# microsoft/Spartan

Measured on AMD Instinct MI355X. Metric: R1CS constraints/sec in SNARK::prove (synthetic 2^20); bit-exact proof, higher is better.
Workload: dtype u64x4 (F_q Montgomery / F_p 2^255-19 limbs)

## Files before the change

### profiles/fq_bandwidth.py

```python
#!/usr/bin/env python3
import csv, sqlite3, sys, collections, re
db = sqlite3.connect(sys.argv[1])
cols = [r[1] for r in db.execute("PRAGMA table_info(kernels)")]
low = {c.lower(): c for c in cols}
def pick(*names):
    for n in names:
        if n in low: return low[n]
    return None
gx, gy, gz = pick("grid_size_x", "grid_x"), pick("grid_size_y", "grid_y"), pick("grid_size_z", "grid_z")
gtot = pick("grid_size")
dcol = low.get("duration") or "(end - start)"
gexpr = gtot if gtot and not gx else "*".join(c for c in (gx, gy, gz) if c)
dur = collections.defaultdict(list)
for name, g, d in db.execute("select name, %s, %s from kernels" % (gexpr, dcol)):
    k = name.split("(")[0].replace("void ", "")
    dur[(k, int(g))].append(d / 1e3)
def load(path, counter):
    tot = collections.defaultdict(float); n = collections.Counter()
    rd = csv.DictReader(open(path))
    gcols = [c for c in rd.fieldnames if c.lower().startswith("grid_size")]
    for row in rd:
        if row["Counter_Name"] != counter: continue
        k = row["Kernel_Name"].split("(")[0].replace("void ", "")
        g = 1
        for c in gcols:
            try: g *= max(1, int(float(row[c])))
            except ValueError: pass
        tot[(k, g)] += float(row["Counter_Value"]); n[(k, g)] += 1
    return tot, n
f, nf = load(sys.argv[2], "FETCH_SIZE"); w, nw = load(sys.argv[3], "WRITE_SIZE")
res = {}
if len(sys.argv) > 4:
    for line in open(sys.argv[4]):
        m = re.match(r"(\S+)\s+vgprs\s+(\d+)\s+waves_per_simd\s+(\d+)", line)
        if m: res[m.group(1)] = (int(m.group(2)), int(m.group(3)))
sq = {}
if len(sys.argv) > 5:
    for c in ("SQ_ACTIVE_INST_VALU", "SQ_WAIT_INST_ANY", "SQ_WAVE_CYCLES"):
        try: sq[c] = load(sys.argv[5], c)
        except OSError: sq = {}; break
def sq_share(k, g, c):
    if not sq: return None
    num, nn = sq[c]; den, nd = sq["SQ_WAVE_CYCLES"]
    if not nn.get((k, g)) or not den.get((k, g)): return None
    return (num[(k, g)] / nn[(k, g)]) / (den[(k, g)] / nd[(k, g)])
FQ = ("k_sc_", "k_cubic_", "k_vecmat", "k_dot", "k_hash_layer", "k_eval_table", "k_sparse_eval", "k_eq_outer", "k_prod_layer", "k_gather", "k_evaluate", "k_spmv", "k_colsum", "k_bind_top", "k_from_index", "k_scale_prefix")
rows = []
for (k, g), ds in dur.items():
    if not k.startswith(FQ): continue
    fb = 2.0 * f.get((k, g), 0.0) * 1024 / max(nf.get((k, g), 1), 1)
    wb = w.get((k, g), 0.0) * 1024 / max(nw.get((k, g), 1), 1)
    avg = sorted(ds)[len(ds) // 2]
    rows.append((k, g, len(ds), avg, fb + wb))
print("# F_q kernels by launch size: HBM bytes per launch (PMC: 2 x FETCH_SIZE + WRITE_SIZE, KiB counters) / median duration (kernel trace)")
print("# throughput-sized = a launch that moves >= 64 MB; the rest is launch-sized (latency-bound by construction: its TB/s says nothing)")
hdr = "%-44s %10s %6s %10s %10s %8s  %-20s %s" % ("kernel", "grid", "calls", "median_us", "MB/launch", "TB/s", "vgprs/waves_per_simd", "valu  wait" if sq else "")
for title, sel in (("throughput-sized launches (>= 64 MB)", lambda r: r[4] >= 64e6), ("launch-sized (< 64 MB), the ten with the most total time", lambda r: r[4] < 64e6)):
    print("\n## " + title); print(hdr)
    part = [r for r in rows if sel(r)]
    part.sort(key=lambda r: -r[2] * r[3])
    if "launch-sized" in title: part = part[:10]
    for k, g, n, avg, b in part:
        base = k.split("<")[0]
        rv = res.get(k) or res.get(base)
        va, wa = sq_share(k, g, "SQ_ACTIVE_INST_VALU"), sq_share(k, g, "SQ_WAIT_INST_ANY")
        tail = ("%.2f  %.2f" % (va, wa)) if (va is not None and wa is not None) else ""
        print("%-44s %10d %6d %10.1f %10.1f %8.2f  %-20s %s" % (k[:44], g, n, avg, b / 1e6, b / avg / 1e6 if avg else 0.0, ("%d / %d" % rv) if rv else "-", tail))
tot_t = sum(r[2] * r[3] for r in rows if r[4] >= 64e6); tot_b = sum(r[2] * r[4] for r in rows if r[4] >= 64e6)
if tot_t: print("\n# all throughput-sized F_q launches together: %.1f ms, %.1f GB -> %.2f TB/s" % (tot_t / 1e3, tot_b / 1e9, tot_b / tot_t / 1e6))
```

### spartan_amd/csrc/field.hpp

```cpp
#pragma once
#include <cstdint>
#include <cstring>

#if defined(__HIPCC__)
#include <hip/hip_runtime.h>
#define SP_HD __host__ __device__ __forceinline__
#define SP_HD_NOINLINE __host__ __device__ __noinline__
#else
#define SP_HD inline
#define SP_HD_NOINLINE
#endif

namespace sp {

typedef unsigned __int128 u128;

struct Fq {
  uint64_t l[4];
};

#define SP_Q0 0x5812631a5cf5d3edULL
#define SP_Q1 0x14def9dea2f79cd6ULL
#define SP_Q2 0x0000000000000000ULL
#define SP_Q3 0x1000000000000000ULL
// ... 262 lines not shown
  }
  constexpr int nprod = i1 - i0 + 1;
  constexpr int nred = (has7 ? 1 : 0) + (K < 8 ? (K < 3 ? K : 3) : (K <= 10 ? 11 - K : 0));
  fq_terms<nprod + nred>(lo, hi, x, y);
  if (K < 8) {
    uint64_t t;
    asm("v_mad_u64_u32 %0, vcc, %1, %2, 0" : "=v"(t) : "v"((uint32_t)lo), "v"((uint32_t)SP_QINV) : "vcc");
    m[K] = (uint32_t)t;
    fq_term1(lo, hi, m[K], q[0]);
  } else {
    r[K - 8] = (uint32_t)lo;
  }
  lo = (lo >> 32) | ((uint64_t)hi << 32);
  hi = 0;
}
__device__ __forceinline__ Fq fq_mul(const Fq& A, const Fq& B) {
  uint32_t a[8], b[8], m[8], r[8];
#pragma unroll
  for (int i = 0; i < 4; i++) {
    a[2 * i] = (uint32_t)A.l[i]; a[2 * i + 1] = (uint32_t)(A.l[i] >> 32);
    b[2 * i] = (uint32_t)B.l[i]; b[2 * i + 1] = (uint32_t)(B.l[i] >> 32);
  }
  const uint32_t q[8] = {(uint32_t)SP_Q0, (uint32_t)(SP_Q0 >> 32), (uint32_t)SP_Q1, (uint32_t)(SP_Q1 >> 32), 0, 0, 0, (uint32_t)(SP_Q3 >> 32)};
  uint64_t lo = 0;
  uint32_t hi = 0;
  fq_column<0>(lo, hi, a, b, m, q, r); fq_column<1>(lo, hi, a, b, m, q, r); fq_column<2>(lo, hi, a, b, m, q, r); fq_column<3>(lo, hi, a, b, m, q, r);
  fq_column<4>(lo, hi, a, b, m, q, r); fq_column<5>(lo, hi, a, b, m, q, r); fq_column<6>(lo, hi, a, b, m, q, r); fq_column<7>(lo, hi, a, b, m, q, r);
  fq_column<8>(lo, hi, a, b, m, q, r); fq_column<9>(lo, hi, a, b, m, q, r); fq_column<10>(lo, hi, a, b, m, q, r); fq_column<11>(lo, hi, a, b, m, q, r);
  fq_column<12>(lo, hi, a, b, m, q, r); fq_column<13>(lo, hi, a, b, m, q, r); fq_column<14>(lo, hi, a, b, m, q, r);
  r[7] = (uint32_t)lo;
  Fq t = {{(uint64_t)r[0] | ((uint64_t)r[1] << 32), (uint64_t)r[2] | ((uint64_t)r[3] << 32), (uint64_t)r[4] | ((uint64_t)r[5] << 32),
           (uint64_t)r[6] | ((uint64_t)r[7] << 32)}};
  return fq_csub(t);
}
__host__ inline Fq fq_mul(const Fq& a, const Fq& b) {
#else
SP_HD Fq fq_mul(const Fq& a, const Fq& b) {
#endif
  uint64_t r[8] = {0, 0, 0, 0, 0, 0, 0, 0};
#pragma unroll
  for (int i = 0; i < 4; i++) {
    u128 c = 0;
#pragma unroll
    for (int j = 0; j < 4; j++) {
      c += (u128)a.l[i] * b.l[j] + r[i + j];
      r[i + j] = (uint64_t)c;
      c >>= 64;
    }
    r[i + 4] = (uint64_t)c;
  }
  return fq_mont_reduce(r);
}
SP_HD Fq fq_sqr(const Fq& a) { return fq_mul(a, a); }
SP_HD Fq fq_from_mont(const Fq& a) {
  uint64_t r[8] = {a.l[0], a.l[1], a.l[2], a.l[3], 0, 0, 0, 0};
  return fq_mont_reduce(r);
}
SP_HD Fq fq_to_mont(const Fq& canonical) { return fq_mul(canonical, fq_R2()); }
SP_HD Fq fq_from_u64(uint64_t v) { return fq_mul(Fq{{v, 0, 0, 0}}, fq_R2()); }
SP_HD Fq fq_from_u512(const uint64_t w[8]) {
  Fq d0 = {{w[0], w[1], w[2], w[3]}}, d1 = {{w[4], w[5], w[6], w[7]}};
  return fq_add(fq_mul(d0, fq_R2()), fq_mul(d1, fq_R3()));
}
SP_HD Fq fq_pow(const Fq& a, const uint64_t e[4]) {
  Fq res = fq_one();
  for (int w = 3; w >= 0; w--)
    for (int i = 63; i >= 0; i--) {
      res = fq_sqr(res);
      if ((e[w] >> i) & 1) res = fq_mul(res, a);
    }
  return res;
}
SP_HD Fq fq_invert(const Fq& a) {
  const uint64_t e[4] = {SP_Q0 - 2, SP_Q1, SP_Q2, SP_Q3};
  return fq_pow(a, e);
}

SP_HD Fq operator+(const Fq& a, const Fq& b) { return fq_add(a, b); }
SP_HD Fq operator-(const Fq& a, const Fq& b) { return fq_sub(a, b); }
SP_HD Fq operator*(const Fq& a, const Fq& b) { return fq_mul(a, b); }
SP_HD Fq operator-(const Fq& a) { return fq_neg(a); }
SP_HD bool operator==(const Fq& a, const Fq& b) { return fq_eq(a, b); }
SP_HD bool operator!=(const Fq& a, const Fq& b) { return !fq_eq(a, b); }
SP_HD Fq& operator+=(Fq& a, const Fq& b) { a = fq_add(a, b); return a; }
SP_HD Fq& operator-=(Fq& a, const Fq& b) { a = fq_sub(a, b); return a; }
SP_HD Fq& operator*=(Fq& a, const Fq& b) { a = fq_mul(a, b); return a; }

struct Fp {
  uint64_t v[4];
};

SP_HD Fp fp_zero() { return Fp{{0, 0, 0, 0}}; }
SP_HD Fp fp_one() { return Fp{{1, 0, 0, 0}}; }

SP_HD uint64_t fp_add_small(Fp& r, uint64_t x) {
  u128 c = (u128)r.v[0] + x;
  r.v[0] = (uint64_t)c;
  c >>= 64;
#pragma unroll
  for (int i = 1; i < 4; i++) {
    c += r.v[i];
    r.v[i] = (uint64_t)c;
    c >>= 64;
  }
  return (uint64_t)c;
}
// ... 270 lines not shown
```

### spartan_amd/csrc/fq_ops.hip

```cpp
#include "internal.hpp"

constexpr int EQ_TOPB = 4;
__device__ __forceinline__ Fq eq_suffix(const Fq* __restrict__ r, size_t ell, int topb, size_t lo) {
  Fq acc = fq_one();
  int nl = (int)ell - topb;
  for (int k = 0; k < nl; k++) {
    Fq rk = ld_fq(r + topb + k);
    bool bit = (lo >> (nl - 1 - k)) & 1;
    acc = fq_mul(acc, bit ? rk : fq_sub(fq_one(), rk));
  }
  return acc;
}
template <int TOPB>
__device__ __forceinline__ void eq_expand_top(Fq (&v)[1 << TOPB], const Fq* __restrict__ r, const Fq& suffix) {
  v[0] = suffix;
#pragma unroll
  for (int k = 0; k < TOPB; k++) {
    Fq rk = ld_fq(r + k);
#pragma unroll
    for (int i = (1 << k) - 1; i >= 0; i--) {
      Fq hi = fq_mul(v[i], rk);
      v[2 * i + 1] = hi;
      v[2 * i] = fq_sub(v[i], hi);
    }
// ... 167 lines not shown
  }
  __syncthreads();
  if (role < 3) {
    Fq e = fq_zero();
    if (live && (KIND == 2 || role < 2)) {
      Fq pt[4];
#pragma unroll
      for (int k = 0; k < NT; k++) {
        Fq x0 = bound[li][2 * k], x1 = bound[li][2 * k + 1];
        Fq x2 = fq_sub(fq_dbl(x1), x0), x3 = fq_sub(fq_add(x2, x1), x0);
#pragma unroll
        for (int w = 0; w < 4; w++) pt[k].l[w] = role == 0 ? x0.l[w] : (role == 1 ? x2.l[w] : x3.l[w]);
      }
      if (KIND == 0) e = fq_mul(pt[0], pt[1]);
      else e = fq_mul(pt[0], fq_sub(fq_mul(pt[1], pt[2]), pt[3]));
    }
    red[role][li] = e;
  }
  __syncthreads();
  for (int s = 16; s > 0; s >>= 1) {
    if (role < 3 && li < s) red[role][li] = fq_add(red[role][li], red[role][li + s]);
    __syncthreads();
  }
  if (threadIdx.x < 3) st_fq(partials + (size_t)blockIdx.x * 3 + threadIdx.x, red[threadIdx.x][0]);
  signal_done(sig);
}
__global__ void __launch_bounds__(256) k_bind_top(Tabs4 T, int ntabs, size_t half, Fq r) { SP_FG_PRIO();
  for (size_t i = (size_t)blockIdx.x * blockDim.x + threadIdx.x; i < half; i += (size_t)gridDim.x * blockDim.x) {
    for (int k = 0; k < ntabs; k++) {
      Fq x0 = ld_fq(T.p[k] + i), x1 = ld_fq(T.p[k] + half + i);
      st_fq(T.p[k] + i, fq_add(x0, fq_mul(r, fq_sub(x1, x0))));
    }
  }
}
__global__ void __launch_bounds__(256) k_reduce_partials(const Fq* __restrict__ partials, size_t nblk, int K, Fq* __restrict__ out, DoneSig sig) { SP_FG_PRIO();
  __shared__ Fq sm[256];
  for (int k = 0; k < K; k++) {
    Fq acc[1] = {fq_zero()};
    for (size_t b = threadIdx.x; b < nblk; b += 256) acc[0] = fq_add(acc[0], ld_fq(partials + b * K + k));
    block_sum_fq<1>(acc, sm);
    if (threadIdx.x == 0) st_fq(out + k, acc[0]);
  }
  signal_done(sig);
}
__global__ void __launch_bounds__(256) k_vecmat(const Fq* __restrict__ L, size_t Lsz, const Fq* __restrict__ Z, size_t R, size_t jchunk,
                                                Fq* __restrict__ partial) { SP_FG_PRIO();
  __shared__ Fq sm[4][64];
  const int cl = threadIdx.x & 63, g = threadIdx.x >> 6;
  size_t i = (size_t)blockIdx.x * 64 + cl;
  size_t j0 = (size_t)blockIdx.y * jchunk, j1 = j0 + jchunk;
  if (j1 > Lsz) j1 = Lsz;
  Fq acc = fq_zero();
  if (i < R)
    for (size_t j = j0 + g; j < j1; j += 4) acc = fq_add(acc, fq_mul(ld_fq(L + j), ld_fq(Z + j * R + i)));
  sm[g][cl] = acc;
  __syncthreads();
  if (g == 0 && i < R) st_fq(partial + (size_t)blockIdx.y * R + i, fq_add(fq_add(sm[0][cl], sm[1][cl]), fq_add(sm[2][cl], sm[3][cl])));
}
__global__ void __launch_bounds__(256) k_colsum(const Fq* __restrict__ partial, size_t nchunks, size_t R, Fq* __restrict__ out) { SP_FG_PRIO();
  __shared__ Fq sm[8][32];
  const int cl = threadIdx.x & 31, g = threadIdx.x >> 5;
  size_t i = (size_t)blockIdx.x * 32 + cl;
  Fq acc = fq_zero();
  if (i < R)
    for (size_t c = g; c < nchunks; c += 8) acc = fq_add(acc, ld_fq(partial + c * R + i));
  sm[g][cl] = acc;
  __syncthreads();
  for (int s = 4; s > 0; s >>= 1) {
    if (g < s) sm[g][cl] = fq_add(sm[g][cl], sm[g + s][cl]);
    __syncthreads();
  }
  if (g == 0 && i < R) st_fq(out + i, sm[0][cl]);
}
static size_t vecmat_jchunk(size_t Lsz, size_t R) { return Lsz * R <= ((size_t)1 << 22) ? 16 : 32; }
__global__ void __launch_bounds__(256) k_dot(const Fq* __restrict__ a, const Fq* __restrict__ b, size_t n, Fq* __restrict__ partials) { SP_FG_PRIO();
  __shared__ Fq sm[256];
  Fq acc[1] = {fq_zero()};
  for (size_t i = (size_t)blockIdx.x * blockDim.x + threadIdx.x; i < n; i += (size_t)gridDim.x * blockDim.x)
    acc[0] = fq_add(acc[0], fq_mul(ld_fq(a + i), ld_fq(b + i)));
  block_sum_fq<1>(acc, sm);
  if (threadIdx.x == 0) st_fq(partials + blockIdx.x, acc[0]);
}
__global__ void k_gather_elems(const Fq* const* __restrict__ ptrs, size_t n, size_t count, Fq* __restrict__ out) { SP_FG_PRIO();
  size_t t = (size_t)blockIdx.x * blockDim.x + threadIdx.x;
  if (t < n * count) st_fq(out + t, ld_fq(ptrs[t / count] + t % count));
}


static void host_sum(const Fq* p, size_t nblk, int K, uint64_t* out) {
  Fq* o = (Fq*)out;
  for (int k = 0; k < K; k++) {
    Fq acc = p[k];
    for (size_t b = 1; b < nblk; b++) acc = fq_add(acc, p[b * K + k]);
    o[k] = acc;
  }
}
int32_t reduce_and_fetch(sp_ctx* c, Fq* partials, size_t nblk, int K, uint64_t* out) {
  if (partials != (Fq*)hres(c)) {
    DoneSig sig = sig_make(c, 1);
    {
      ProfScope ps(c, PF_REDUCE, 32.0 * (double)(nblk * K));
      hipLaunchKernelGGL(k_reduce_partials, dim3(1), dim3(256), 0, c->stream, (const Fq*)partials, nblk, K, (Fq*)hres(c), sig);
    }
    SPCHK(sig_wait(c, sig));
    memcpy(out, hres(c), 32 * K);
    return hipGetLastError() == hipSuccess ? SP_OK : SP_EHIP;
  }
// ... 446 lines not shown
```

### spartan_amd/csrc/internal.hpp

```cpp
#pragma once
#include <hip/hip_runtime.h>

#include <cstdio>
#include <cstdlib>
#include <cstring>
#include <new>
#include <map>
#include <vector>

#include "../../include/spartan_hip.h"
#include "curve.hpp"
#include "field.hpp"
#include "msm.hpp"
#include "options.hpp"

using namespace sp;

enum ProfFamily {
  PF_GENS_TABLE = 0,
  PF_MSM_ROWS,
  PF_MSM_WINDOWS,
  PF_MSM_REDUCE_PASS,
  PF_MSM_REDUCE,
  PF_EQ_EXPAND,
// ... 234 lines not shown
int32_t reduce_and_fetch(sp_ctx* c, Fq* partials, size_t nblk, int K, uint64_t* out);
constexpr size_t SP_HOST_ENCODE_ROWS = 8;
extern "C" int32_t msm_launch(sp_ctx* c, const sp_gens* g, const Fq* dZ, size_t z_stride, size_t rows, size_t cols, size_t g_off,
                              const uint32_t* didx, const Fq* dblinds, size_t h_idx, uint8_t* out_host, size_t idx_row_stride = 0,
                              Pt* points_out = nullptr );

enum MsmRowsForm { MSM_ROWS_WINDOWS = 0, MSM_ROWS_STRIP, MSM_ROWS_FLAT };
size_t msm_flat_slots();
void msm_rows_enqueue(sp_ctx* c, hipStream_t st, const sp_gens* g, const Fq* dZ, size_t z_stride, size_t rows, size_t cols, size_t g_off,
                      const uint32_t* didx, const Fq* dblinds, size_t h_idx, Pt* partial, int form, size_t strip, size_t P);

size_t msm_lds_runs(const sp_gens* g, size_t rows, size_t cols, bool has_blinds, size_t wg_slots);
void msm_lds_enqueue(sp_ctx* c, hipStream_t st, const sp_gens* g, const Fq* dZ, size_t z_stride, size_t rows, size_t cols, size_t g_off,
                     const uint32_t* didx, const Fq* dblinds, size_t h_idx, Pt* partial, size_t nb, unsigned grid_limit);

struct MsmQRuns { unsigned nb, len, S; };
constexpr unsigned MSMQ_MAX_GROUPS = 1024, MSMQ_BLOCK_WORDS = 2 * MSMQ_MAX_GROUPS + 2 , MSMQ_BLOCKS = 256;
enum MsmQRole { MSMQ_ALONE = 0, MSMQ_CORESIDENT = 2 };
MsmQRuns msm_q_cut(const sp_ctx* c, const sp_gens* g, size_t rows, size_t cols, bool has_blinds, int role);
void msm_q_enqueue(sp_ctx* c, hipStream_t st, const sp_gens* g, const Fq* dZ, size_t z_stride, size_t rows, size_t cols, size_t g_off,
                   const uint32_t* didx, const Fq* dblinds, size_t h_idx, Pt* partial, const MsmQRuns& r, int role,
                   const unsigned** counts_out ,
                   const unsigned long long** issued_out );

static inline size_t grid_for(size_t work, size_t maxblocks = 2048) {
  size_t b = (work + 255) / 256;
  if (b < 1) b = 1;
  return b > maxblocks ? maxblocks : b;
}
static inline bool is_pow2(size_t x) { return x && !(x & (x - 1)); }
static inline size_t ilog2(size_t x) {
  size_t l = 0;
  while (((size_t)1 << l) < x) l++;
  return l;
}

#ifndef SP_FG_PRIO_OFF
#define SP_FG_PRIO() __builtin_amdgcn_s_setprio(3)
#else
#define SP_FG_PRIO() do { } while (0)
#endif

__device__ __forceinline__ Fq ld_fq(const Fq* p) {
  const ulonglong2* q = reinterpret_cast<const ulonglong2*>(p);
  ulonglong2 a = q[0], b = q[1];
  return Fq{{a.x, a.y, b.x, b.y}};
}
__device__ __forceinline__ void st_fq(Fq* p, const Fq& v) {
  ulonglong2* q = reinterpret_cast<ulonglong2*>(p);
  q[0] = make_ulonglong2(v.l[0], v.l[1]);
  q[1] = make_ulonglong2(v.l[2], v.l[3]);
}

template <int K>
__device__ __forceinline__ void block_sum_fq(Fq (&v)[K], Fq* smem ) {
  int t = threadIdx.x;
#pragma unroll
  for (int k = 0; k < K; k++) {
    __syncthreads();
    smem[t] = v[k];
    __syncthreads();
    for (int s = 128; s > 0; s >>= 1) {
      if (t < s) smem[t] = fq_add(smem[t], smem[t + s]);
      __syncthreads();
    }
    v[k] = smem[0];
  }
}


__global__ void k_reduce_partials(const Fq* __restrict__ partials, size_t nblk, int K, Fq* __restrict__ out);
```

### spartan_amd/csrc/spark.hip

```cpp
#include "internal.hpp"

__global__ void __launch_bounds__(256) k_from_index(const uint32_t* __restrict__ ix, size_t n, Fq* __restrict__ dst) { SP_FG_PRIO();
  for (size_t i = (size_t)blockIdx.x * blockDim.x + threadIdx.x; i < n; i += (size_t)gridDim.x * blockDim.x) st_fq(dst + i, fq_from_u64(ix[i]));
}
__global__ void __launch_bounds__(256) k_gather(const Fq* __restrict__ mem, const uint32_t* __restrict__ addr, size_t n, Fq* __restrict__ dst) { SP_FG_PRIO();
  for (size_t i = (size_t)blockIdx.x * blockDim.x + threadIdx.x; i < n; i += (size_t)gridDim.x * blockDim.x) st_fq(dst + i, ld_fq(mem + addr[i]));
}
__global__ void __launch_bounds__(256) k_hash_layer(const Fq* __restrict__ addr, const Fq* __restrict__ val, const Fq* __restrict__ ts, int ts_inc,
                                                    size_t n, Fq r_hash, Fq r_hash_sqr, Fq r_multiset, Fq* __restrict__ dst) { SP_FG_PRIO();
  for (size_t i = (size_t)blockIdx.x * blockDim.x + threadIdx.x; i < n; i += (size_t)gridDim.x * blockDim.x) {
    Fq a = addr ? ld_fq(addr + i) : fq_from_u64((uint64_t)i);
    Fq t = ts ? ld_fq(ts + i) : fq_zero();
    if (ts_inc) t = fq_add(t, fq_one());
    Fq h = fq_add(fq_add(fq_mul(t, r_hash_sqr), fq_mul(ld_fq(val + i), r_hash)), a);
    st_fq(dst + i, fq_sub(h, r_multiset));
  }
}
template <bool PAIR>
__global__ void __launch_bounds__(256) k_hash_layer_first(const Fq* __restrict__ addr, const Fq* __restrict__ val, const Fq* __restrict__ ts, int ts_inc,
                                                          size_t n, Fq r_hash, Fq r_hash_sqr, Fq r_multiset, Fq* __restrict__ dst_a, Fq* __restrict__ dst_b) { SP_FG_PRIO();
  const size_t half = n / 2;
  for (size_t i = (size_t)blockIdx.x * blockDim.x + threadIdx.x; i < half; i += (size_t)gridDim.x * blockDim.x) {
    Fq h[2];
#pragma unroll
    for (int k = 0; k < 2; k++) {
      const size_t j = i + (size_t)k * half;
      Fq a = addr ? ld_fq(addr + j) : fq_from_u64((uint64_t)j);
      Fq t = ts ? ld_fq(ts + j) : fq_zero();
      if (ts_inc) t = fq_add(t, fq_one());
      h[k] = fq_sub(fq_add(fq_add(fq_mul(t, r_hash_sqr), fq_mul(ld_fq(val + j), r_hash)), a), r_multiset);
      st_fq(dst_a + j, h[k]);
    }
    st_fq(dst_a + n + i, fq_mul(h[0], h[1]));
    if (PAIR) {
      Fq w0 = fq_add(h[0], r_hash_sqr), w1 = fq_add(h[1], r_hash_sqr);
      st_fq(dst_b + i, w0);
      st_fq(dst_b + half + i, w1);
      st_fq(dst_b + n + i, fq_mul(w0, w1));
    }
  }
}
__global__ void __launch_bounds__(256) k_prod_layer(const Fq* __restrict__ in, size_t half, Fq* __restrict__ out) { SP_FG_PRIO();
  for (size_t i = (size_t)blockIdx.x * blockDim.x + threadIdx.x; i < half; i += (size_t)gridDim.x * blockDim.x)
    st_fq(out + i, fq_mul(ld_fq(in + i), ld_fq(in + half + i)));
}

struct Stores16 {
  Fq* p[16];
};
__global__ void __launch_bounds__(256) k_prod_layer_many(Stores16 st, size_t off, size_t half, size_t noff) { SP_FG_PRIO();
  const Fq* in = st.p[blockIdx.y] + off;
  Fq* out = st.p[blockIdx.y] + noff;
  for (size_t i = (size_t)blockIdx.x * blockDim.x + threadIdx.x; i < half; i += (size_t)gridDim.x * blockDim.x)
    st_fq(out + i, fq_mul(ld_fq(in + i), ld_fq(in + half + i)));
}

__global__ void __launch_bounds__(256) k_prod_layer2_many(Stores16 st, size_t off, size_t len) { SP_FG_PRIO();
  const size_t q = len / 4, off1 = off + len, off2 = off1 + len / 2;
  Fq* base = st.p[blockIdx.y];
  for (size_t i = (size_t)blockIdx.x * blockDim.x + threadIdx.x; i < q; i += (size_t)gridDim.x * blockDim.x) {
    const Fq x0 = ld_fq(base + off + i), x1 = ld_fq(base + off + q + i), x2 = ld_fq(base + off + 2 * q + i), x3 = ld_fq(base + off + 3 * q + i);
    const Fq lo = fq_mul(x0, x2), hi = fq_mul(x1, x3);
    st_fq(base + off1 + i, lo);
    st_fq(base + off1 + q + i, hi);
    st_fq(base + off2 + i, fq_mul(lo, hi));
  }
}
__global__ void __launch_bounds__(256) k_prod_layer_tail(Stores16 st, size_t off, size_t len) { SP_FG_PRIO();
  __shared__ Fq cur[1024];
  Fq* base = st.p[blockIdx.x];
  size_t half = len / 2, noff = off + len;
  for (size_t i = threadIdx.x; i < half; i += 256) {
    Fq v = fq_mul(ld_fq(base + off + i), ld_fq(base + off + half + i));
    cur[i] = v;
    st_fq(base + noff + i, v);
  }
  __syncthreads();
  len = half;
  while (len > 2) {
    half = len / 2;
    noff += len;
    Fq v[2];
    int n = 0;
// ... 14 lines not shown
__device__ __forceinline__ void cubic_point(const Fq& a0, const Fq& a1, const Fq& b0, const Fq& b1, const Fq& c0, const Fq& c1, Fq (&e)[3]) {
  Fq da = fq_sub(a1, a0), db = fq_sub(b1, b0), dc = fq_sub(c1, c0);
  Fq a2 = fq_add(a1, da), b2 = fq_add(b1, db), c2 = fq_add(c1, dc);
  Fq a3 = fq_add(a2, da), b3 = fq_add(b2, db), c3 = fq_add(c2, dc);
  e[0] = fq_add(e[0], fq_mul(fq_mul(a0, b0), c0));
  e[1] = fq_add(e[1], fq_mul(fq_mul(a2, b2), c2));
  e[2] = fq_add(e[2], fq_mul(fq_mul(a3, b3), c3));
}
__global__ void __launch_bounds__(256) k_cubic_eval_batched(const Triple* __restrict__ T, TripleInline IN, size_t half, Fq* __restrict__ partials) { SP_FG_PRIO();
  __shared__ Fq sm[256];
  Triple t = T ? T[blockIdx.y] : IN.t[blockIdx.y];
  Fq e[3] = {fq_zero(), fq_zero(), fq_zero()};
  for (size_t i = (size_t)blockIdx.x * blockDim.x + threadIdx.x; i < half; i += (size_t)gridDim.x * blockDim.x)
    cubic_point(ld_fq(t.a + i), ld_fq(t.a + half + i), ld_fq(t.b + i), ld_fq(t.b + half + i), ld_fq(t.c + i), ld_fq(t.c + half + i), e);
  block_sum_fq<3>(e, sm);
  if (threadIdx.x == 0) {
    Fq* p = partials + ((size_t)blockIdx.y * gridDim.x + blockIdx.x) * 3;
    st_fq(p, e[0]); st_fq(p + 1, e[1]); st_fq(p + 2, e[2]);
  }
}
__global__ void __launch_bounds__(256) k_cubic_bind_eval_batched(const Triple* __restrict__ T, TripleInline IN, size_t quarter, Fq r, Fq* __restrict__ partials) { SP_FG_PRIO();
  __shared__ Fq sm[256];
  Triple t = T ? T[blockIdx.y] : IN.t[blockIdx.y];
  Fq e[3] = {fq_zero(), fq_zero(), fq_zero()};
  for (size_t i = (size_t)blockIdx.x * blockDim.x + threadIdx.x; i < quarter; i += (size_t)gridDim.x * blockDim.x) {
    Fq lo[3], hi[3];
    Fq* ptr[3] = {t.a, t.b, t.c};
#pragma unroll
    for (int k = 0; k < 3; k++) {
      Fq x0 = ld_fq(ptr[k] + i), x1 = ld_fq(ptr[k] + quarter + i), x2 = ld_fq(ptr[k] + 2 * quarter + i), x3 = ld_fq(ptr[k] + 3 * quarter + i);
      lo[k] = fq_add(x0, fq_mul(r, fq_sub(x2, x0)));
      hi[k] = fq_add(x1, fq_mul(r, fq_sub(x3, x1)));
      if (k < 2) {
        st_fq(ptr[k] + i, lo[k]);
        st_fq(ptr[k] + quarter + i, hi[k]);
      } else if (t.c_out) {
        st_fq(t.c_out + i, lo[k]);
        st_fq(t.c_out + quarter + i, hi[k]);
      }
    }
    cubic_point(lo[0], hi[0], lo[1], hi[1], lo[2], hi[2], e);
  }
  block_sum_fq<3>(e, sm);
  if (threadIdx.x == 0) {
    Fq* p = partials + ((size_t)blockIdx.y * gridDim.x + blockIdx.x) * 3;
    st_fq(p, e[0]); st_fq(p + 1, e[1]); st_fq(p + 2, e[2]);
  }
}
__device__ __forceinline__ void quad_point_eq(const Fq& a0, const Fq& a1, const Fq& b0, const Fq& b1, const Fq& c, Fq (&e)[4]) {
  Fq a2 = fq_add(a1, fq_sub(a1, a0)), b2 = fq_add(b1, fq_sub(b1, b0));
  e[0] = fq_add(e[0], fq_mul(fq_mul(a0, b0), c));
  e[1] = fq_add(e[1], fq_mul(fq_mul(a2, b2), c));
}
__device__ __forceinline__ void cubic_point4(const Fq& a0, const Fq& a1, const Fq& b0, const Fq& b1, const Fq& c0, const Fq& c1, Fq (&e)[4]) {
  Fq da = fq_sub(a1, a0), db = fq_sub(b1, b0), dc = fq_sub(c1, c0);
  Fq a2 = fq_add(a1, da), b2 = fq_add(b1, db), c2 = fq_add(c1, dc);
  Fq a3 = fq_add(a2, da), b3 = fq_add(b2, db), c3 = fq_add(c2, dc);
  e[0] = fq_add(e[0], fq_mul(fq_mul(a0, b0), c0));
  e[1] = fq_add(e[1], fq_mul(fq_mul(a1, b1), c1));
  e[2] = fq_add(e[2], fq_mul(fq_mul(a2, b2), c2));
  e[3] = fq_add(e[3], fq_mul(fq_mul(a3, b3), c3));
}
template <bool GEN>
__global__ void __launch_bounds__(256) k_cubic_eval_batched_eq(TripleInline IN, unsigned inst0, size_t half, Fq* __restrict__ partials) { SP_FG_PRIO();
  __shared__ Fq sm[256];
  const unsigned inst = inst0 + blockIdx.y;
  Triple t = IN.t[inst];
  Fq e[4] = {fq_zero(), fq_zero(), fq_zero(), fq_zero()};
  if (!GEN) {
    for (size_t i = (size_t)blockIdx.x * blockDim.x + threadIdx.x; i < half; i += (size_t)gridDim.x * blockDim.x)
      quad_point_eq(ld_fq(t.a + i), ld_fq(t.a + half + i), ld_fq(t.b + i), ld_fq(t.b + half + i), ld_fq(t.c + i), e);
  } else {
    for (size_t i = (size_t)blockIdx.x * blockDim.x + threadIdx.x; i < half; i += (size_t)gridDim.x * blockDim.x)
      cubic_point4(ld_fq(t.a + i), ld_fq(t.a + half + i), ld_fq(t.b + i), ld_fq(t.b + half + i), ld_fq(t.c + i), ld_fq(t.c + half + i), e);
  }
  if (GEN) block_sum_fq<4>(e, sm);
  else {
    Fq q[2] = {e[0], e[1]};
    block_sum_fq<2>(q, sm);
    e[0] = q[0]; e[1] = q[1];
  }
  if (threadIdx.x == 0) {
    Fq* p = partials + ((size_t)inst * gridDim.x + blockIdx.x) * 4;
    st_fq(p, e[0]); st_fq(p + 1, e[1]); st_fq(p + 2, e[2]); st_fq(p + 3, e[3]);
  }
}
template <bool GEN>
__global__ void __launch_bounds__(256) k_cubic_bind_eval_batched_eq(TripleInline IN, unsigned inst0, size_t quarter, Fq r, Fq* __restrict__ partials) { SP_FG_PRIO();
  __shared__ Fq sm[256];
  const unsigned inst = inst0 + blockIdx.y;
  Triple t = IN.t[inst];
  Fq e[4] = {fq_zero(), fq_zero(), fq_zero(), fq_zero()};
  for (size_t i = (size_t)blockIdx.x * blockDim.x + threadIdx.x; i < quarter; i += (size_t)gridDim.x * blockDim.x) {
    Fq lo[3], hi[3];
    Fq* ptr[3] = {t.a, t.b, t.c};
#pragma unroll
    for (int k = 0; k < 2; k++) {
      Fq x0 = ld_fq(ptr[k] + i), x1 = ld_fq(ptr[k] + quarter + i), x2 = ld_fq(ptr[k] + 2 * quarter + i), x3 = ld_fq(ptr[k] + 3 * quarter + i);
      lo[k] = fq_add(x0, fq_mul(r, fq_sub(x2, x0)));
      hi[k] = fq_add(x1, fq_mul(r, fq_sub(x3, x1)));
      st_fq(ptr[k] + i, lo[k]);
      st_fq(ptr[k] + quarter + i, hi[k]);
    }
    if (!GEN) {
      quad_point_eq(lo[0], hi[0], lo[1], hi[1], ld_fq(t.c + i), e);
    } else {
      Fq x0 = ld_fq(ptr[2] + i), x1 = ld_fq(ptr[2] + quarter + i), x2 = ld_fq(ptr[2] + 2 * quarter + i), x3 = ld_fq(ptr[2] + 3 * quarter + i);
      lo[2] = fq_add(x0, fq_mul(r, fq_sub(x2, x0)));
      hi[2] = fq_add(x1, fq_mul(r, fq_sub(x3, x1)));
      if (t.c_out) {
        st_fq(t.c_out + i, lo[2]);
        st_fq(t.c_out + quarter + i, hi[2]);
      }
      cubic_point4(lo[0], hi[0], lo[1], hi[1], lo[2], hi[2], e);
    }
  }
  if (GEN) block_sum_fq<4>(e, sm);
  else {
    Fq q[2] = {e[0], e[1]};
    block_sum_fq<2>(q, sm);
    e[0] = q[0]; e[1] = q[1];
  }
  if (threadIdx.x == 0) {
    Fq* p = partials + ((size_t)inst * gridDim.x + blockIdx.x) * 4;
// ... 150 lines not shown
    const int k = lane / 3, tt = lane % 3;
    const Fq P = lv[grp][k][2][tt], U = lv[grp][k][3][tt];
    lv[grp][k][4][tt] = fq_add(P, U);
    lv[grp][k][5][tt] = fq_sub(P, U);
  }
  __syncthreads();
  Fq e = fq_zero();
  if (live && lane < 18 && np >= 2) {
    const int tt = lane / 6, kind = lane % 6;
    if (kind == 0 || np == 4) {
      e = fq_mul(fq_mul(lv[grp][0][kind][tt], lv[grp][1][kind][tt]), lv[grp][2][kind][tt]);
      SP_KT(kt, 4);
      if (weights) e = fq_mul(e, wv);
    }
  }
  SP_KT(kt, 5);
  if (lane < 18) red[lane][grp] = e;
  __syncthreads();
  if (threadIdx.x < 18) {
    Fq acc = red[threadIdx.x][0];
#pragma unroll
    for (int k = 1; k < 8; k++) acc = fq_add(acc, red[threadIdx.x][k]);
    red[threadIdx.x][0] = acc;
  }
  __syncthreads();
  if (threadIdx.x < 18) {
    Fq* o = partials + ((size_t)blockIdx.y * gridDim.x + blockIdx.x) * 18;
    const int x = threadIdx.x;
    Fq v;
    if (x < 3) v = fq_add(red[6 * x][0], red[6 * x + 1][0]);
    else if (x < 15) v = red[6 * ((x - 3) / 4) + 2 + (x - 3) % 4][0];
    else v = (n2 == 1 && blockIdx.x == 0) ? bnd[0][(x - 15) * 4] : fq_zero();
    st_fq(o + x, v);
  }
  SP_KT(kt, 6);
  signal_done(sig);
  SP_KT(kt, 7);
}
__global__ void __launch_bounds__(256) k_reduce_partials_batched(const Fq* __restrict__ partials, size_t nblk, int K, Fq* __restrict__ out, DoneSig sig) { SP_FG_PRIO();
  __shared__ Fq sm[256];
  const Fq* p = partials + (size_t)blockIdx.x * nblk * K;
  for (int k = 0; k < K; k++) {
    Fq acc[1] = {fq_zero()};
    for (size_t b = threadIdx.x; b < nblk; b += 256) acc[0] = fq_add(acc[0], ld_fq(p + b * K + k));
    block_sum_fq<1>(acc, sm);
    if (threadIdx.x == 0) st_fq(out + (size_t)blockIdx.x * K + k, acc[0]);
  }
  signal_done(sig);
}
__global__ void __launch_bounds__(256) k_dot_many(const Fq* __restrict__ chi, Fq* const* __restrict__ tabs, size_t n, Fq* __restrict__ partials) { SP_FG_PRIO();
  __shared__ Fq sm[256];
  const Fq* t = tabs[blockIdx.y];
  Fq acc[1] = {fq_zero()};
  for (size_t i = (size_t)blockIdx.x * blockDim.x + threadIdx.x; i < n; i += (size_t)gridDim.x * blockDim.x)
    acc[0] = fq_add(acc[0], fq_mul(ld_fq(chi + i), ld_fq(t + i)));
  block_sum_fq<1>(acc, sm);
  if (threadIdx.x == 0) st_fq(partials + (size_t)blockIdx.y * gridDim.x + blockIdx.x, acc[0]);
}
__global__ void __launch_bounds__(256) k_dot3(const Fq* __restrict__ l, const Fq* __restrict__ r, const Fq* __restrict__ w, size_t n,
                                              Fq* __restrict__ partials) { SP_FG_PRIO();
  __shared__ Fq sm[256];
  Fq acc[1] = {fq_zero()};
  for (size_t i = (size_t)blockIdx.x * blockDim.x + threadIdx.x; i < n; i += (size_t)gridDim.x * blockDim.x)
    acc[0] = fq_add(acc[0], fq_mul(fq_mul(ld_fq(l + i), ld_fq(r + i)), ld_fq(w + i)));
  block_sum_fq<1>(acc, sm);
  if (threadIdx.x == 0) st_fq(partials + blockIdx.x, acc[0]);
}

__global__ void __launch_bounds__(256) k_dot3_many(const Fq* const* __restrict__ ptrs, size_t nt, size_t n, Fq* __restrict__ partials) { SP_FG_PRIO();
  __shared__ Fq sm[256];
  const Fq *l = ptrs[blockIdx.y], *r = ptrs[nt + blockIdx.y], *w = ptrs[2 * nt + blockIdx.y];
  Fq acc[1] = {fq_zero()};
  for (size_t i = (size_t)blockIdx.x * blockDim.x + threadIdx.x; i < n; i += (size_t)gridDim.x * blockDim.x)
    acc[0] = fq_add(acc[0], fq_mul(fq_mul(ld_fq(l + i), ld_fq(r + i)), ld_fq(w + i)));
  block_sum_fq<1>(acc, sm);
  if (threadIdx.x == 0) st_fq(partials + (size_t)blockIdx.y * gridDim.x + blockIdx.x, acc[0]);
}

static Fq limbs(const uint64_t* p) {
  Fq x;
  memcpy(x.l, p, 32);
  return x;
}

extern "C" {

int32_t sp_index_upload(sp_ctx* c, const uint64_t* idx, size_t n, sp_index** out) {
  if (!c || !idx || !out || n == 0) return SP_EINVAL;
  std::vector<uint32_t> v(n);
  for (size_t i = 0; i < n; i++) {
    if (idx[i] > 0xffffffffULL) return SP_EINVAL;
    v[i] = (uint32_t)idx[i];
  }
  HIPCHK(hipSetDevice(c->dev));
  sp_index* ix = new (std::nothrow) sp_index();
  if (!ix) return SP_ENOMEM;
  ix->ctx = c; ix->n = n; ix->d = nullptr;
  hipError_t e = hipMalloc((void**)&ix->d, 4 * n);
  if (e == hipSuccess) e = hipMemcpy(ix->d, v.data(), 4 * n, hipMemcpyHostToDevice);
  if (e != hipSuccess) { if (ix->d) (void)hipFree(ix->d); delete ix; return e == hipErrorOutOfMemory ? SP_ENOMEM : SP_EHIP; }
  *out = ix;
  return SP_OK;
}
void sp_index_free(sp_index* ix) {
  if (!ix) return;
  (void)hipSetDevice(ix->ctx->dev);
  (void)hipStreamSynchronize(ix->ctx->stream);
  (void)hipFree(ix->d);
  delete ix;
}
int32_t sp_table_from_index(sp_ctx* c, const sp_index* ix, sp_table* dst, size_t dst_off) {
  if (!c || !ix || !dst || dst_off + ix->n > dst->cap) return SP_EINVAL;
  HIPCHK(hipSetDevice(c->dev));
  ProfScope ps(c, PF_SPARK, 36.0 * (double)ix->n);
  hipLaunchKernelGGL(k_from_index, dim3((unsigned)grid_for(ix->n)), dim3(256), 0, c->stream, (const uint32_t*)ix->d, ix->n, dst->d + dst_off);
  return hipGetLastError() == hipSuccess ? SP_OK : SP_EHIP;
}
int32_t sp_table_view(sp_ctx* c, const sp_table* parent, size_t off, size_t len, sp_table** out) {
  if (!c || !parent || !out || len == 0 || off + len > parent->cap) return SP_EINVAL;
  sp_table* t = new (std::nothrow) sp_table();
  if (!t) return SP_ENOMEM;
  t->ctx = c; t->d = parent->d + off; t->cap = t->len = len; t->owner = 0; t->d_bytes = 0; t->alt = nullptr; t->alt_bytes = 0;
  *out = t;
  return SP_OK;
}
int32_t sp_gather(sp_ctx* c, const sp_table* mem, const sp_index* addr, sp_table* dst, size_t dst_off) {
  if (!c || !mem || !addr || !dst || dst_off + addr->n > dst->cap) return SP_EINVAL;
// ... 512 lines not shown
```

Baseline: 47.52 million.

## Accumulate products unreduced in wide 512-bit accumulators, reduce once per batch

Adds an FqWide 512-bit accumulator with a 32-bit-limb multiply-accumulate and a separate Montgomery reduction. The dot-product, vecmat, cubic-eval and hash-leaf kernels now sum up to FQ_WIDE_FLUSH products before reducing once, instead of reducing every product. This removes most per-term Montgomery reductions from these reduction-heavy kernels. In exchange it raises register pressure from the 16-word accumulator, which may cost occupancy or cause scratch spills. It also adds a profiling script that compares kernel durations and resource usage.

```diff
diff --git a/profiles/fq_bandwidth.py b/profiles/fq_bandwidth.py
--- a/profiles/fq_bandwidth.py
+++ b/profiles/fq_bandwidth.py
@@ -32,7 +32,7 @@
 res = {}
 if len(sys.argv) > 4:
     for line in open(sys.argv[4]):
-        m = re.match(r"(\S+)\s+vgprs\s+(\d+)\s+waves_per_simd\s+(\d+)", line)
+        m = re.match(r"(\S+)\s+vgprs\s+(\d+)\s+(?:scratch\s+\d+\s+)?waves_per_simd\s+(\d+)", line)
         if m: res[m.group(1)] = (int(m.group(2)), int(m.group(3)))
 sq = {}
 if len(sys.argv) > 5:
diff --git a/profiles/fq_wide_kernel_stats.py b/profiles/fq_wide_kernel_stats.py
--- /dev/null
+++ b/profiles/fq_wide_kernel_stats.py
@@ -0,0 +1,58 @@
+#!/usr/bin/env python3
+import collections, re, sqlite3, sys
+
+
+def durations(path):
+    db = sqlite3.connect(path)
+    cols = {r[1].lower(): r[1] for r in db.execute("PRAGMA table_info(kernels)")}
+    g = ("*".join(cols[c] for c in ("grid_size_x", "grid_size_y", "grid_size_z") if c in cols) or "*".join(cols[c] for c in ("grid_x", "grid_y", "grid_z") if c in cols)
+         or cols["grid_size"])
+    d = cols.get("duration") or "(end - start)"
+    out = collections.defaultdict(list)
+    for name, grid, dur in db.execute("select name, %s, %s from kernels" % (g, d)):
+        out[(name.split("(")[0].replace("void ", ""), int(grid))].append(dur / 1e3)
+    return out
+
+
+def resources(path):
+    res = {}
+    for line in open(path):
+        m = re.match(r"(\S+)\s+vgprs\s+(\d+)\s+(?:scratch\s+(\d+)\s+)?waves_per_simd\s+(\d+)", line)
+        if m:
+            res[m.group(1)] = "%s/%s/%s" % (m.group(2), m.group(3) or "-", m.group(4))
+    return res
+
+
+parent, result = durations(sys.argv[1]), durations(sys.argv[2])
+big = set()
+for line in open(sys.argv[3]):
+    if line.startswith("## launch-sized"):
+        break
+    f = line.split()
+    if len(f) >= 5 and f[0].startswith("k_") and f[1].isdigit():
+        big.add((f[0], int(f[1])))
+rp = resources(sys.argv[4]) if len(sys.argv) > 4 else {}
+rr = resources(sys.argv[5]) if len(sys.argv) > 5 else {}
+med = lambda v: sorted(v)[len(v) // 2]
+FQ = ("k_sc_", "k_cubic_", "k_vecmat", "k_dot", "k_hash_layer", "k_eval_table", "k_sparse_eval", "k_evaluate", "k_spmv")
+CONVERTED = ("k_cubic_eval_batched_eq<false>", "k_hash_layer", "k_dot_many", "k_dot3", "k_vecmat")
+print("# median launch duration (us) by kernel and launch size, parent | result; vgprs/scratch/waves_per_simd from kernel_resources.sh")
+print("%-40s %9s %6s %10s %10s %8s  %-12s %-12s %s" % ("kernel", "grid", "calls", "parent_us", "result_us", "change", "parent_res", "result_res", "wide"))
+tot = {"p": 0.0, "r": 0.0}
+rows = []
+for key in sorted(set(parent) & set(result)):
+    k, g = key
+    if not k.startswith(FQ) or key not in big:
+        continue
+    n = min(len(parent[key]), len(result[key]))
+    p, r = med(parent[key]), med(result[key])
+    rows.append((n * p, k, g, n, p, r))
+    tot["p"] += n * p; tot["r"] += n * r
+for _, k, g, n, p, r in sorted(rows, reverse=True):
+    conv = "yes" if k.startswith(CONVERTED) and not k.endswith("_tiny") else ""
+    print("%-40s %9d %6d %10.1f %10.1f %7.1f%%  %-12s %-12s %s" % (k[:40], g, n, p, r, 100.0 * (r / p - 1), rp.get(k, "-"), rr.get(k, "-"), conv))
+print("\n# all throughput-sized F_q launches together (calls x median): parent %.2f ms, result %.2f ms (%.1f%%)" % (
+    tot["p"] / 1e3, tot["r"] / 1e3, 100.0 * (tot["r"] / tot["p"] - 1) if tot["p"] else 0.0))
+only = sorted(k for k in (set(parent) ^ set(result)) if k[0].startswith(FQ) and k in big)
+if only:
+    print("# launch classes present in one trace only: %s" % only)
diff --git a/spartan_amd/csrc/field.hpp b/spartan_amd/csrc/field.hpp
--- a/spartan_amd/csrc/field.hpp
+++ b/spartan_amd/csrc/field.hpp
@@ -338,6 +338,166 @@
   return fq_mont_reduce(r);
 }
 SP_HD Fq fq_sqr(const Fq& a) { return fq_mul(a, a); }
+
+struct FqWide {
+  uint64_t l[8];
+};
+#define FQ_WIDE_MAX_TERMS 15
+static_assert((u128)FQ_WIDE_MAX_TERMS * ((u128)SP_Q3 + 1) <= (u128)0xffffffffffffffffULL, "FQ_WIDE_MAX_TERMS * q < 2^256: that many products of residues stay below q * 2^256");
+SP_HD FqWide fq_wide_zero() { return FqWide{{0, 0, 0, 0, 0, 0, 0, 0}}; }
+
+#if defined(__HIP_DEVICE_COMPILE__) && !defined(SP_FQ_MUL_GENERIC)
+__device__ __forceinline__ void fq_wide_split(const FqWide& a, uint32_t (&w)[16]) {
+#pragma unroll
+  for (int i = 0; i < 8; i++) { w[2 * i] = (uint32_t)a.l[i]; w[2 * i + 1] = (uint32_t)(a.l[i] >> 32); }
+}
+__device__ __forceinline__ void fq_wide_join(FqWide& a, const uint32_t (&w)[16]) {
+#pragma unroll
+  for (int i = 0; i < 8; i++) a.l[i] = (uint64_t)w[2 * i] | ((uint64_t)w[2 * i + 1] << 32);
+}
+template <int K>
+__device__ __forceinline__ void fq_mac_column(uint64_t& lo, uint32_t& hi, const uint32_t (&a)[8], const uint32_t (&b)[8], uint32_t (&w)[16]) {
+  constexpr int i0 = K < 8 ? 0 : K - 7, i1 = K < 8 ? K : 7;
+  uint32_t x[16], y[16];
+  int n = 0;
+#pragma unroll
+  for (int i = i0; i <= i1; i++) { x[n] = a[i]; y[n] = b[K - i]; n++; }
+  lo += (uint64_t)w[K];
+  fq_terms<i1 - i0 + 1>(lo, hi, x, y);
+  w[K] = (uint32_t)lo;
+  lo = (lo >> 32) | ((uint64_t)hi << 32);
+  hi = 0;
+}
+__device__ __forceinline__ void fq_mac_wide(FqWide& acc, const Fq& A, const Fq& B) {
+  uint32_t a[8], b[8], w[16];
+#pragma unroll
+  for (int i = 0; i < 4; i++) {
+    a[2 * i] = (uint32_t)A.l[i]; a[2 * i + 1] = (uint32_t)(A.l[i] >> 32);
+    b[2 * i] = (uint32_t)B.l[i]; b[2 * i + 1] = (uint32_t)(B.l[i] >> 32);
+  }
+  fq_wide_split(acc, w);
+  uint64_t lo = 0;
+  uint32_t hi = 0;
+  fq_mac_column<0>(lo, hi, a, b, w); fq_mac_column<1>(lo, hi, a, b, w); fq_mac_column<2>(lo, hi, a, b, w); fq_mac_column<3>(lo, hi, a, b, w);
+  fq_mac_column<4>(lo, hi, a, b, w); fq_mac_column<5>(lo, hi, a, b, w); fq_mac_column<6>(lo, hi, a, b, w); fq_mac_column<7>(lo, hi, a, b, w);
+  fq_mac_column<8>(lo, hi, a, b, w); fq_mac_column<9>(lo, hi, a, b, w); fq_mac_column<10>(lo, hi, a, b, w); fq_mac_column<11>(lo, hi, a, b, w);
+  fq_mac_column<12>(lo, hi, a, b, w); fq_mac_column<13>(lo, hi, a, b, w); fq_mac_column<14>(lo, hi, a, b, w);
+  w[15] += (uint32_t)lo;
+  fq_wide_join(acc, w);
+}
+__device__ __forceinline__ void fq_mac_wide_u64(FqWide& acc, const Fq& A, uint64_t k) {
+  uint32_t a[8], w[16];
+#pragma unroll
+  for (int i = 0; i < 4; i++) { a[2 * i] = (uint32_t)A.l[i]; a[2 * i + 1] = (uint32_t)(A.l[i] >> 32); }
+  fq_wide_split(acc, w);
+  const uint32_t k0 = (uint32_t)k, k1 = (uint32_t)(k >> 32);
+  uint64_t lo = 0;
+  uint32_t hi = 0;
+#pragma unroll
+  for (int K = 0; K < 9; K++) {
+    lo += (uint64_t)w[K];
+    if (K >= 1 && K < 8) fq_term2(lo, hi, a[K], k0, a[K - 1], k1);
+    else if (K == 0) fq_term1(lo, hi, a[0], k0);
+    else fq_term1(lo, hi, a[7], k1);
+    w[K] = (uint32_t)lo;
+    lo = (lo >> 32) | ((uint64_t)hi << 32);
+    hi = 0;
+  }
+#pragma unroll
+  for (int K = 9; K < 16; K++) {
+    lo += (uint64_t)w[K];
+    w[K] = (uint32_t)lo;
+    lo >>= 32;
+  }
+  fq_wide_join(acc, w);
+}
+template <int K>
+__device__ __forceinline__ void fq_redc_column(uint64_t& lo, uint32_t& hi, const uint32_t (&w)[16], uint32_t (&m)[8], const uint32_t (&q)[8],
+                                               uint32_t (&r)[8]) {
+  constexpr bool has7 = K >= 7;
+  constexpr int j0 = K < 8 ? (K >= 3 ? K - 3 : 0) : (K - 3 > K - 7 ? K - 3 : K - 7);
+  uint32_t x[16], y[16];
+  int n = 0;
+  if (has7) { x[n] = m[K - 7]; y[n] = q[7]; n++; }
+#pragma unroll
+  for (int i = j0; i <= 7; i++) {
+    const int v = K - i;
+    if (v >= (K < 8 ? 1 : 0) && v <= 3) { x[n] = m[i]; y[n] = q[v]; n++; }
+  }
+  constexpr int nred = (has7 ? 1 : 0) + (K < 8 ? (K < 3 ? K : 3) : (K <= 10 ? 11 - K : 0));
+  lo += (uint64_t)w[K];
+  if constexpr (nred > 0) fq_terms<nred>(lo, hi, x, y);
+  if (K < 8) {
+    uint64_t t;
+    asm("v_mad_u64_u32 %0, vcc, %1, %2, 0" : "=v"(t) : "v"((uint32_t)lo), "v"((uint32_t)SP_QINV) : "vcc");
+    m[K] = (uint32_t)t;
+    fq_term1(lo, hi, m[K], q[0]);
+  } else {
+    r[K - 8] = (uint32_t)lo;
+  }
+  lo = (lo >> 32) | ((uint64_t)hi << 32);
+  hi = 0;
+}
+__device__ __forceinline__ Fq fq_redc_wide(const FqWide& acc) {
+  uint32_t w[16], m[8], r[8];
+  fq_wide_split(acc, w);
+  const uint32_t q[8] = {(uint32_t)SP_Q0, (uint32_t)(SP_Q0 >> 32), (uint32_t)SP_Q1, (uint32_t)(SP_Q1 >> 32), 0, 0, 0, (uint32_t)(SP_Q3 >> 32)};
+  uint64_t lo = 0;
+  uint32_t hi = 0;
+  fq_redc_column<0>(lo, hi, w, m, q, r); fq_redc_column<1>(lo, hi, w, m, q, r); fq_redc_column<2>(lo, hi, w, m, q, r); fq_redc_column<3>(lo, hi, w, m, q, r);
+  fq_redc_column<4>(lo, hi, w, m, q, r); fq_redc_column<5>(lo, hi, w, m, q, r); fq_redc_column<6>(lo, hi, w, m, q, r); fq_redc_column<7>(lo, hi, w, m, q, r);
+  fq_redc_column<8>(lo, hi, w, m, q, r); fq_redc_column<9>(lo, hi, w, m, q, r); fq_redc_column<10>(lo, hi, w, m, q, r); fq_redc_column<11>(lo, hi, w, m, q, r);
+  fq_redc_column<12>(lo, hi, w, m, q, r); fq_redc_column<13>(lo, hi, w, m, q, r); fq_redc_column<14>(lo, hi, w, m, q, r);
+  r[7] = (uint32_t)lo + w[15];
+  Fq t = {{(uint64_t)r[0] | ((uint64_t)r[1] << 32), (uint64_t)r[2] | ((uint64_t)r[3] << 32), (uint64_t)r[4] | ((uint64_t)r[5] << 32),
+           (uint64_t)r[6] | ((uint64_t)r[7] << 32)}};
+  return fq_csub(t);
+}
+__host__ inline void fq_mac_wide(FqWide& acc, const Fq& a, const Fq& b) {
+#else
+SP_HD void fq_mac_wide(FqWide& acc, const Fq& a, const Fq& b) {
+#endif
+#pragma unroll
+  for (int i = 0; i < 4; i++) {
+    u128 c = 0;
+#pragma unroll
+    for (int j = 0; j < 4; j++) {
+      c += (u128)a.l[i] * b.l[j] + acc.l[i + j];
+      acc.l[i + j] = (uint64_t)c;
+      c >>= 64;
+    }
+#pragma unroll
+    for (int j = i + 4; j < 8; j++) {
+      c += acc.l[j];
+      acc.l[j] = (uint64_t)c;
+      c >>= 64;
+    }
+  }
+}
+#if defined(__HIP_DEVICE_COMPILE__) && !defined(SP_FQ_MUL_GENERIC)
+__host__ inline void fq_mac_wide_u64(FqWide& acc, const Fq& a, uint64_t k) {
+#else
+SP_HD void fq_mac_wide_u64(FqWide& acc, const Fq& a, uint64_t k) {
+#endif
+  u128 c = 0;
+#pragma unroll
+  for (int j = 0; j < 4; j++) {
+    c += (u128)a.l[j] * k + acc.l[j];
+    acc.l[j] = (uint64_t)c;
+    c >>= 64;
+  }
+#pragma unroll
+  for (int j = 4; j < 8; j++) {
+    c += acc.l[j];
+    acc.l[j] = (uint64_t)c;
+    c >>= 64;
+  }
+}
+#if defined(__HIP_DEVICE_COMPILE__) && !defined(SP_FQ_MUL_GENERIC)
+__host__ inline Fq fq_redc_wide(const FqWide& acc) { return fq_mont_reduce(acc.l); }
+#else
+SP_HD Fq fq_redc_wide(const FqWide& acc) { return fq_mont_reduce(acc.l); }
+#endif
 SP_HD Fq fq_from_mont(const Fq& a) {
   uint64_t r[8] = {a.l[0], a.l[1], a.l[2], a.l[3], 0, 0, 0, 0};
   return fq_mont_reduce(r);
diff --git a/spartan_amd/csrc/fq_ops.hip b/spartan_amd/csrc/fq_ops.hip
--- a/spartan_amd/csrc/fq_ops.hip
+++ b/spartan_amd/csrc/fq_ops.hip
@@ -243,7 +243,11 @@
   if (j1 > Lsz) j1 = Lsz;
   Fq acc = fq_zero();
   if (i < R)
-    for (size_t j = j0 + g; j < j1; j += 4) acc = fq_add(acc, fq_mul(ld_fq(L + j), ld_fq(Z + j * R + i)));
+    for (size_t j = j0 + g; j < j1;) {
+      FqWide w = fq_wide_zero();
+      for (int t = 0; t < FQ_WIDE_FLUSH && j < j1; t++, j += 4) fq_mac_wide(w, ld_fq(L + j), ld_fq(Z + j * R + i));
+      acc = fq_add(acc, fq_redc_wide(w));
+    }
   sm[g][cl] = acc;
   __syncthreads();
   if (g == 0 && i < R) st_fq(partial + (size_t)blockIdx.y * R + i, fq_add(fq_add(sm[0][cl], sm[1][cl]), fq_add(sm[2][cl], sm[3][cl])));
diff --git a/spartan_amd/csrc/internal.hpp b/spartan_amd/csrc/internal.hpp
--- a/spartan_amd/csrc/internal.hpp
+++ b/spartan_amd/csrc/internal.hpp
@@ -310,6 +310,9 @@
   q[1] = make_ulonglong2(v.l[2], v.l[3]);
 }
 
+constexpr int FQ_WIDE_FLUSH = 8;
+static_assert(FQ_WIDE_FLUSH >= 1 && FQ_WIDE_FLUSH <= FQ_WIDE_MAX_TERMS, "a wide accumulator holds at most FQ_WIDE_MAX_TERMS products of residues");
+
 template <int K>
 __device__ __forceinline__ void block_sum_fq(Fq (&v)[K], Fq* smem ) {
   int t = threadIdx.x;
diff --git a/spartan_amd/csrc/spark.hip b/spartan_amd/csrc/spark.hip
--- a/spartan_amd/csrc/spark.hip
+++ b/spartan_amd/csrc/spark.hip
@@ -5,15 +5,25 @@
 }
 __global__ void __launch_bounds__(256) k_gather(const Fq* __restrict__ mem, const uint32_t* __restrict__ addr, size_t n, Fq* __restrict__ dst) { SP_FG_PRIO();
   for (size_t i = (size_t)blockIdx.x * blockDim.x + threadIdx.x; i < n; i += (size_t)gridDim.x * blockDim.x) st_fq(dst + i, ld_fq(mem + addr[i]));
+}
+__device__ __forceinline__ Fq hash_leaf(const Fq* __restrict__ addr, const Fq* __restrict__ val, const Fq* __restrict__ ts, int ts_inc, size_t j,
+                                        const Fq& r_hash, const Fq& r_hash_sqr, const Fq& r_multiset) {
+  FqWide w = fq_wide_zero();
+  if (ts || ts_inc) {
+    Fq t = ts ? ld_fq(ts + j) : fq_zero();
+    if (ts_inc) t = fq_add(t, fq_one());
+    fq_mac_wide(w, t, r_hash_sqr);
+  }
+  fq_mac_wide(w, ld_fq(val + j), r_hash);
+  if (!addr) fq_mac_wide_u64(w, fq_R2(), (uint64_t)j);
+  Fq h = fq_redc_wide(w);
+  if (addr) h = fq_add(h, ld_fq(addr + j));
+  return fq_sub(h, r_multiset);
 }
 __global__ void __launch_bounds__(256) k_hash_layer(const Fq* __restrict__ addr, const Fq* __restrict__ val, const Fq* __restrict__ ts, int ts_inc,
                                                     size_t n, Fq r_hash, Fq r_hash_sqr, Fq r_multiset, Fq* __restrict__ dst) { SP_FG_PRIO();
   for (size_t i = (size_t)blockIdx.x * blockDim.x + threadIdx.x; i < n; i += (size_t)gridDim.x * blockDim.x) {
-    Fq a = addr ? ld_fq(addr + i) : fq_from_u64((uint64_t)i);
-    Fq t = ts ? ld_fq(ts + i) : fq_zero();
-    if (ts_inc) t = fq_add(t, fq_one());
-    Fq h = fq_add(fq_add(fq_mul(t, r_hash_sqr), fq_mul(ld_fq(val + i), r_hash)), a);
-    st_fq(dst + i, fq_sub(h, r_multiset));
+    st_fq(dst + i, hash_leaf(addr, val, ts, ts_inc, i, r_hash, r_hash_sqr, r_multiset));
   }
 }
 template <bool PAIR>
@@ -25,10 +35,7 @@
 #pragma unroll
     for (int k = 0; k < 2; k++) {
       const size_t j = i + (size_t)k * half;
-      Fq a = addr ? ld_fq(addr + j) : fq_from_u64((uint64_t)j);
-      Fq t = ts ? ld_fq(ts + j) : fq_zero();
-      if (ts_inc) t = fq_add(t, fq_one());
-      h[k] = fq_sub(fq_add(fq_add(fq_mul(t, r_hash_sqr), fq_mul(ld_fq(val + j), r_hash)), a), r_multiset);
+      h[k] = hash_leaf(addr, val, ts, ts_inc, j, r_hash, r_hash_sqr, r_multiset);
       st_fq(dst_a + j, h[k]);
     }
     st_fq(dst_a + n + i, fq_mul(h[0], h[1]));
@@ -149,6 +156,11 @@
   e[0] = fq_add(e[0], fq_mul(fq_mul(a0, b0), c));
   e[1] = fq_add(e[1], fq_mul(fq_mul(a2, b2), c));
 }
+__device__ __forceinline__ void quad_point_eq_wide(const Fq& a0, const Fq& a1, const Fq& b0, const Fq& b1, const Fq& c, FqWide& w0, FqWide& w1) {
+  Fq a2 = fq_add(a1, fq_sub(a1, a0)), b2 = fq_add(b1, fq_sub(b1, b0));
+  fq_mac_wide(w0, fq_mul(a0, b0), c);
+  fq_mac_wide(w1, fq_mul(a2, b2), c);
+}
 __device__ __forceinline__ void cubic_point4(const Fq& a0, const Fq& a1, const Fq& b0, const Fq& b1, const Fq& c0, const Fq& c1, Fq (&e)[4]) {
   Fq da = fq_sub(a1, a0), db = fq_sub(b1, b0), dc = fq_sub(c1, c0);
   Fq a2 = fq_add(a1, da), b2 = fq_add(b1, db), c2 = fq_add(c1, dc);
@@ -165,8 +177,14 @@
   Triple t = IN.t[inst];
   Fq e[4] = {fq_zero(), fq_zero(), fq_zero(), fq_zero()};
   if (!GEN) {
-    for (size_t i = (size_t)blockIdx.x * blockDim.x + threadIdx.x; i < half; i += (size_t)gridDim.x * blockDim.x)
-      quad_point_eq(ld_fq(t.a + i), ld_fq(t.a + half + i), ld_fq(t.b + i), ld_fq(t.b + half + i), ld_fq(t.c + i), e);
+    const size_t stride = (size_t)gridDim.x * blockDim.x;
+    for (size_t i = (size_t)blockIdx.x * blockDim.x + threadIdx.x; i < half;) {
+      FqWide w0 = fq_wide_zero(), w1 = fq_wide_zero();
+      for (int g = 0; g < FQ_WIDE_FLUSH && i < half; g++, i += stride)
+        quad_point_eq_wide(ld_fq(t.a + i), ld_fq(t.a + half + i), ld_fq(t.b + i), ld_fq(t.b + half + i), ld_fq(t.c + i), w0, w1);
+      e[0] = fq_add(e[0], fq_redc_wide(w0));
+      e[1] = fq_add(e[1], fq_redc_wide(w1));
+    }
   } else {
     for (size_t i = (size_t)blockIdx.x * blockDim.x + threadIdx.x; i < half; i += (size_t)gridDim.x * blockDim.x)
       cubic_point4(ld_fq(t.a + i), ld_fq(t.a + half + i), ld_fq(t.b + i), ld_fq(t.b + half + i), ld_fq(t.c + i), ld_fq(t.c + half + i), e);
@@ -423,8 +441,12 @@
   __shared__ Fq sm[256];
   const Fq* t = tabs[blockIdx.y];
   Fq acc[1] = {fq_zero()};
-  for (size_t i = (size_t)blockIdx.x * blockDim.x + threadIdx.x; i < n; i += (size_t)gridDim.x * blockDim.x)
-    acc[0] = fq_add(acc[0], fq_mul(ld_fq(chi + i), ld_fq(t + i)));
+  const size_t stride = (size_t)gridDim.x * blockDim.x;
+  for (size_t i = (size_t)blockIdx.x * blockDim.x + threadIdx.x; i < n;) {
+    FqWide w = fq_wide_zero();
+    for (int g = 0; g < FQ_WIDE_FLUSH && i < n; g++, i += stride) fq_mac_wide(w, ld_fq(chi + i), ld_fq(t + i));
+    acc[0] = fq_add(acc[0], fq_redc_wide(w));
+  }
   block_sum_fq<1>(acc, sm);
   if (threadIdx.x == 0) st_fq(partials + (size_t)blockIdx.y * gridDim.x + blockIdx.x, acc[0]);
 }
@@ -432,8 +454,12 @@
                                               Fq* __restrict__ partials) { SP_FG_PRIO();
   __shared__ Fq sm[256];
   Fq acc[1] = {fq_zero()};
-  for (size_t i = (size_t)blockIdx.x * blockDim.x + threadIdx.x; i < n; i += (size_t)gridDim.x * blockDim.x)
-    acc[0] = fq_add(acc[0], fq_mul(fq_mul(ld_fq(l + i), ld_fq(r + i)), ld_fq(w + i)));
+  const size_t stride = (size_t)gridDim.x * blockDim.x;
+  for (size_t i = (size_t)blockIdx.x * blockDim.x + threadIdx.x; i < n;) {
+    FqWide s = fq_wide_zero();
+    for (int g = 0; g < FQ_WIDE_FLUSH && i < n; g++, i += stride) fq_mac_wide(s, fq_mul(ld_fq(l + i), ld_fq(r + i)), ld_fq(w + i));
+    acc[0] = fq_add(acc[0], fq_redc_wide(s));
+  }
   block_sum_fq<1>(acc, sm);
   if (threadIdx.x == 0) st_fq(partials + blockIdx.x, acc[0]);
 }
@@ -442,8 +468,12 @@
   __shared__ Fq sm[256];
   const Fq *l = ptrs[blockIdx.y], *r = ptrs[nt + blockIdx.y], *w = ptrs[2 * nt + blockIdx.y];
   Fq acc[1] = {fq_zero()};
-  for (size_t i = (size_t)blockIdx.x * blockDim.x + threadIdx.x; i < n; i += (size_t)gridDim.x * blockDim.x)
-    acc[0] = fq_add(acc[0], fq_mul(fq_mul(ld_fq(l + i), ld_fq(r + i)), ld_fq(w + i)));
+  const size_t stride = (size_t)gridDim.x * blockDim.x;
+  for (size_t i = (size_t)blockIdx.x * blockDim.x + threadIdx.x; i < n;) {
+    FqWide s = fq_wide_zero();
+    for (int g = 0; g < FQ_WIDE_FLUSH && i < n; g++, i += stride) fq_mac_wide(s, fq_mul(ld_fq(l + i), ld_fq(r + i)), ld_fq(w + i));
+    acc[0] = fq_add(acc[0], fq_redc_wide(s));
+  }
   block_sum_fq<1>(acc, sm);
   if (threadIdx.x == 0) st_fq(partials + (size_t)blockIdx.y * gridDim.x + blockIdx.x, acc[0]);
 }
```

Result: faster. 48.31 million, median of 6 (+1.7%).
